# facebookresearch/FlowDec

Hardware: AMD Instinct MI355X
Metric: 48 kHz audio-seconds/sec (RTF) for FlowDec-75m @ 6 ODE steps (higher is better)
Workload: dtype bf16; 1 GPU; flowdec_75m enhance(): global batch=8 x 2 s clips @48 kHz (8 per GPU), 6-step euler (NFE 6), T_pad=256 frames, inputs resident in HBM, initial noise drawn inside the timed call, output waveforms all-gathered; global_batch=8, nfe=6, parallelism=batch-shard x1, hipgraph=True, conv_algo=auto

## Files before the change

flowdec_amd/csrc/conv_wino4.hip:

```cpp
#include <type_traits>

#include "conv_common.h"
#include "wino4_layout.h"

namespace {

using namespace fdconv;

typedef _Float16 f16;
typedef __attribute__((ext_vector_type(2))) _Float16 f16x2;
typedef __attribute__((ext_vector_type(8))) _Float16 f16x8;
typedef unsigned int u32x2 __attribute__((ext_vector_type(2)));
typedef float f32x2 __attribute__((ext_vector_type(2)));

constexpr int cmax(int a, int b) { return a > b ? a : b; }

using fdw4::NTH, fdw4::HH, fdw4::HW, fdw4::RROW, fdw4::RROW_BYTES, fdw4::RAW_PASSES, fdw4::RAW_BYTES, fdw4::NPIECE, fdw4::VXI;
constexpr int TH = 16, TW = 16, BN = 256;
static_assert(HH == TH + 2 && HW == TW + 2, "wino4_layout.h describes this tile");
constexpr int CK = 16;
constexpr int SLAB = BN * 32;
constexpr int RSLOT = 2048, NRING = 6;
static_assert(18 % NRING == 0, "the two-chunk loop body turns the ring a whole number of times");
constexpr int RING_BYTES = 8 * NRING * RSLOT;
constexpr int V_BYTES = 6 * VXI;
constexpr int V_OFF = RING_BYTES;
constexpr int AFF_OFF = V_OFF + 2 * V_BYTES;
constexpr int RAW_OFF = AFF_OFF + AFF_BYTES;
constexpr int MAIN_BYTES = RAW_OFF + RAW_BYTES;
constexpr int X_BYTES = 8 * 8192;
constexpr int S_PITCH = 128 * 4 + 16;
constexpr int S_BYTES = 128 * S_PITCH;
constexpr int SK_OFF = S_BYTES, SK_BYTES = 4 * NTH * 16;
constexpr int SCK = 2, SCD = 3;
constexpr int WS_BYTES = SCK * SLAB;
constexpr int XS_OFF = SCD * WS_BYTES, XS_BYTES = SCK * 8192;
constexpr int BIAS_OFF = 2 * S_BYTES;
static_assert(BIAS_OFF >= 2 * X_BYTES && BIAS_OFF >= SK_OFF + 2 * SK_BYTES && XS_OFF + SCD * XS_BYTES <= 160 * 1024, "epilogue LDS map");
constexpr int ISC_OFF = BIAS_OFF + 1024;
constexpr int STAT_OFF = ISC_OFF + 1024;
constexpr int LDS_BYTES = cmax(MAIN_BYTES, STAT_OFF + 16384);
static_assert(LDS_BYTES <= 160 * 1024 && NPIECE <= RAW_PASSES * NTH && AFF_BYTES <= 4 * 1024 && RAW_OFF % 128 == 0, "LDS layout");
constexpr int U_EXP = 9;
constexpr float RAW_MAX = 6000.f;

__device__ __forceinline__ unsigned pack_f16(float a, float b) {
  f16x2 r = {(f16)a, (f16)b};
  return __builtin_bit_cast(unsigned, r);
}
__device__ __forceinline__ f16x2 h2(unsigned u) { return __builtin_bit_cast(f16x2, u); }
__device__ __forceinline__ unsigned u2(f16x2 v) { return __builtin_bit_cast(unsigned, v); }

__device__ __forceinline__ void glds16s(const void* sbase, unsigned voff, unsigned lds_dst) {
  asm volatile("s_mov_b32 m0, %2\n\ts_nop 0\n\tglobal_load_lds_dwordx4 %0, %1" ::"v"(voff), "s"(sbase), "s"(lds_dst) : "memory");
}
__device__ __forceinline__ void glds16s_x2(const void* sbase, unsigned voff, unsigned lds_dst) {
  asm volatile("s_mov_b32 m0, %2\n\ts_nop 0\n\tglobal_load_lds_dwordx4 %0, %1\n\tglobal_load_lds_dwordx4 %0, %1 offset:1024" ::"v"(voff), "s"(sbase), "s"(lds_dst)
               : "memory");
}

template <bool ACT, bool SKIP, bool SC>
__global__ __launch_bounds__(NTH, 2) void conv_wino4_kernel(ConvArgs p) {
  static_assert(!(SKIP && SC), "residual input and folded shortcut exclude each other in this kernel");
  extern __shared__ __attribute__((aligned(16))) char smem[];
  FD_T2(const unsigned long long t2_entry = __builtin_amdgcn_s_memtime();)

  const int bid = blockIdx.x, nblk = gridDim.x;
  int lid;
  {
    const int xcd = bid & 7, qq = nblk >> 3, rr = nblk & 7;
    lid = (xcd < rr ? xcd * (qq + 1) : rr * (qq + 1) + (xcd - rr) * qq) + (bid >> 3);
  }
  if (p.reversed) lid = nblk - 1 - lid;
  int pt = lid;
  const int tw_i = pt % p.tiles_w; pt /= p.tiles_w;
  const int th_i = pt % p.tiles_h;
  const int b = pt / p.tiles_h;
  const int h0 = th_i * TH, w0 = tw_i * TW;
  const int H = p.H, W = p.W;

  const int t = threadIdx.x;
  const int lane = t & 63;
  const int wave = __builtin_amdgcn_readfirstlane(t >> 6);
  const int cq = wave & 3, xt = wave >> 2;

  auto opaque = [&](int v) { asm volatile("" : "+v"(v)); return v; };
  const size_t img_elems = (size_t)H * W;
  const int hb = h0 > 0 ? h0 - 1 : 0;
  const size_t band_pix = (size_t)b * img_elems + (size_t)hb * W;
  const bf16* const sb0 = reinterpret_cast<const bf16*>(p.seg[0].src) + band_pix * p.seg[0].C;
  const bool two3 = p.nseg > 1 && p.seg[1].taps == 9;
  const bf16* const sb1 = two3 ? reinterpret_cast<const bf16*>(p.seg[1].src) + band_pix * p.seg[1].C : sb0;
  const int sC0 = p.seg[0].C, sC1 = two3 ? p.seg[1].C : 0;
  const int nch0 = sC0 / CK, n3 = nch0 + sC1 / CK;
  int hpix[RAW_PASSES];
#pragma unroll
  for (int i = 0; i < RAW_PASSES; ++i) {
    const fdw4::Req rq = fdw4::raw_request(t + i * NTH);
    const int gh = h0 - 1 + rq.row, gw = w0 - 1 + rq.col;
    const bool ok = rq.col >= 0 && gh >= 0 && gh < H && gw >= 0 && gw < W;
    hpix[i] = ((ok ? (gh - hb) * W + gw : 0) << 2) | (ok ? rq.piece : t & 3);
  }
  int pA, vbits, pword;
  {
    const fdw4::Item it = fdw4::item(t);
    pA = fdw4::raw_addr(it.row, 6 * it.k, 0, it.word) | (fdw4::v_addr(it.row, fdw4::first_tile(it.k), it.word) << 16);
    const int gh = h0 - 1 + it.row;
    vbits = (it.k != 0 || w0 > 0 ? 1 : 0) | (gh >= 0 && gh < H ? 2 : 0) | (it.k != 2 || w0 + TW < W ? 4 : 0) | (it.active ? 8 : 0) |
            (it.active && it.k == 1 ? 16 : 0);
    pword = it.word;
  }
  const bf16* nbase = sb0;
  int nC2 = 0, ncb = 0;
  int cnext = 0;
  auto next_chunk = [&]() {
    if (cnext < n3) {
      const bool first = cnext < nch0;
      const int cch = first ? cnext : cnext - nch0;
      nbase = first ? sb0 : sb1;
      nC2 = (first ? sC0 : sC1) * 2;
      ncb = cch * CK * 2;
    }
    ++cnext;
  };
  const unsigned rawdst = (unsigned)(RAW_OFF + wave * 1024);
  auto load_halo = [&]() {
    const int on = cnext <= n3 ? 1 : 0;
#pragma unroll
    for (int i = 0; i < RAW_PASSES; ++i) {
      const int hp = opaque(hpix[i]);
      glds16s(nbase, (unsigned)(((hp >> 2) * nC2 + ncb + (hp & 3) * 16) * on), rawdst + i * 8192);
    }
  };
  int affa = AFF_OFF + pword * 16;
  auto load_affine = [&]() {
    if constexpr (ACT) {
      if (wave < AFF_BYTES / 1024) {
        const int o = opaque(t) * 16;
        glds16s(p.affine + (size_t)b * p.affC * 2, (unsigned)(o < n3 * CK * 8 ? o : 0), (unsigned)(AFF_OFF + wave * 1024));
      }
    }
  };

  auto produce = [&](const int e, const int vbuf, const int affo) {
    const int pa = opaque(pA), vbt = opaque(vbits);
    const char* const rp = smem + RAW_OFF + ((pa & 0xffff) ^ (e << 5));
    char* const vb = smem + V_OFF + vbuf * V_BYTES + (int)((unsigned)pa >> 16);
    unsigned w_[6];
#pragma unroll
    for (int j = 0; j < 6; ++j) w_[j] = *reinterpret_cast<const unsigned*>(rp + j * 64);
    f32x4 af = {0.f, 0.f, 0.f, 0.f};
    if constexpr (ACT) af = *reinterpret_cast<const f32x4*>(smem + opaque(affa) + affo);
    const unsigned mrow = (unsigned)((int)((unsigned)vbt << 30) >> 31);
    const unsigned m0 = mrow & (unsigned)((int)((unsigned)vbt << 31) >> 31), m5 = mrow & (unsigned)((int)((unsigned)vbt << 29) >> 31);
#pragma unroll
    for (int j = 0; j < 6; ++j) {
      const unsigned u = w_[j];
      const float x0 = __builtin_bit_cast(float, u << 16), x1 = __builtin_bit_cast(float, u & 0xffff0000u);
      unsigned r;
      if constexpr (ACT) {
        const f16x2 zc = {(f16)RAW_MAX, (f16)RAW_MAX};
        r = u2(__builtin_elementwise_min(h2(pack_f16(fd_silu(fmaf(x0, af[0], af[1])), fd_silu(fmaf(x1, af[2], af[3])))), zc));
      } else
        r = pack_f16(__builtin_amdgcn_fmed3f(x0, -RAW_MAX, RAW_MAX), __builtin_amdgcn_fmed3f(x1, -RAW_MAX, RAW_MAX));
      w_[j] = r & (j == 0 ? m0 : j == 5 ? m5 : mrow);
    }
    const unsigned l4 = (unsigned)__builtin_amdgcn_update_dpp(0, (int)w_[4], 0x111, 0xf, 0xf, true);
    const unsigned l5 = (unsigned)__builtin_amdgcn_update_dpp(0, (int)w_[5], 0x111, 0xf, 0xf, true);
    const unsigned r0 = (unsigned)__builtin_amdgcn_update_dpp(0, (int)w_[0], 0x101, 0xf, 0xf, true);
    const unsigned r1 = (unsigned)__builtin_amdgcn_update_dpp(0, (int)w_[1], 0x101, 0xf, 0xf, true);
    const bool mid = (vbt & 16) != 0;
    const f16x2 c4 = {(f16)4.f, (f16)4.f}, cm4 = {(f16)-4.f, (f16)-4.f}, cm5 = {(f16)-5.f, (f16)-5.f}, c2 = {(f16)2.f, (f16)2.f},
                cm2 = {(f16)-2.f, (f16)-2.f};
    auto transform = [&](char* const v, const unsigned d0, const unsigned d1, const unsigned d2, const unsigned d3, const unsigned d4, const unsigned d5) {
      const f16x2 z0 = h2(d0), z1 = h2(d1), z2 = h2(d2), z3 = h2(d3), z4 = h2(d4), z5 = h2(d5);
      const f16x2 t1 = __builtin_elementwise_fma(z2, cm4, z4);
      const f16x2 t2 = __builtin_elementwise_fma(z1, cm4, z3);
      const f16x2 t3 = z4 - z2, t4 = z3 - z1;
      *reinterpret_cast<unsigned*>(v + 0 * VXI) = u2(__builtin_elementwise_fma(z0, c4, __builtin_elementwise_fma(z2, cm5, z4)));
      *reinterpret_cast<unsigned*>(v + 1 * VXI) = u2(t1 + t2);
      *reinterpret_cast<unsigned*>(v + 2 * VXI) = u2(t1 - t2);
      *reinterpret_cast<unsigned*>(v + 4 * VXI) = u2(__builtin_elementwise_fma(t4, c2, t3));
      *reinterpret_cast<unsigned*>(v + 5 * VXI) = u2(__builtin_elementwise_fma(t4, cm2, t3));
      *reinterpret_cast<unsigned*>(v + 3 * VXI) = u2(__builtin_elementwise_fma(z1, c4, __builtin_elementwise_fma(z3, cm5, z5)));
    };
    if (vbt & 8)
      transform(vb, mid ? l4 : w_[0], mid ? l5 : w_[1], mid ? w_[0] : w_[2], mid ? w_[1] : w_[3], mid ? w_[2] : w_[4], mid ? w_[3] : w_[5]);
    if (mid) transform(vb + 32, w_[2], w_[3], w_[4], w_[5], r0, r1);
  };

  const char* wp = reinterpret_cast<const char*>(p.w) + (size_t)xt * 9 * SLAB + cq * 2048;
  asm volatile("" : "+s"(wp));
  const unsigned lane16 = (unsigned)(lane * 16);
  const unsigned wring = (unsigned)(wave * NRING * RSLOT);
  auto dma_step = [&](int f, int slot) {
    glds16s_x2(wp + (f / 9) * 18 * SLAB + (f % 9) * SLAB, lane16, wring + slot * RSLOT);
  };

  const int l31 = lane & 31, lh = lane >> 5;
  const int wa_lane = (int)wring + l31 * 32 + ((lh ^ ((l31 >> 3) & 1)) * 16);
  const int vb0 = V_OFF + xt * 3 * VXI  + l31 * 32 + ((lh ^ ((l31 >> 3) & 1)) * 16);
  const int vb1 = (vb0 ^ ((l31 & 4) << 2)) + 128;

  f32x16 acc[3][2][2];
#pragma unroll
  for (int x = 0; x < 3; ++x)
#pragma unroll
    for (int ct = 0; ct < 2; ++ct)
#pragma unroll
      for (int nt = 0; nt < 2; ++nt)
#pragma unroll
        for (int e = 0; e < 16; ++e) acc[x][ct][nt][e] = 0.f;

  auto lds_wait = [&]() { asm volatile("s_waitcnt lgkmcnt(0)" ::: "memory"); };
  auto barrier = [&]() {
    __builtin_amdgcn_s_barrier();
    asm volatile("" ::: "memory");
  };

  u32x4 qa[3], qb[3];
  auto mma = [&](int xl, int ct, int nt, const u32x4& a, const u32x4& bq) {
    acc[xl][ct][nt] = __builtin_amdgcn_mfma_f32_32x32x16_f16(__builtin_bit_cast(f16x8, a), __builtin_bit_cast(f16x8, bq), acc[xl][ct][nt], 0, 0, 0);
  };
  auto rd = [&](int off) { return *reinterpret_cast<const u32x4*>(smem + off); };
  auto a_off = [&](int k18, int ct) { return wa_lane + (k18 % NRING) * RSLOT + ct * 1024; };
  auto b_off = [&](int k18, int nt) {
    const int s = k18 % 9, half = (k18 / 9) & 1;
    const int dy = s % 3;
    return (dy == 0 ? vb0 : dy == 1 ? vb1 : (vb0 ^ 16) + 256) + half * V_BYTES + (s / 3) * VXI + nt * 1024;
  };

  next_chunk();
  load_halo();
  load_affine();
#pragma unroll
  for (int k = 0; k < NRING; ++k) dma_step(k, k);
  asm volatile("s_waitcnt vmcnt(0)" ::: "memory");
  barrier();
  produce(0, 0, 0);
  next_chunk();
  lds_wait();
  barrier();
  FD_T2(const unsigned long long t2_first = __builtin_amdgcn_s_memtime();)
  qa[0] = rd(a_off(0, 0)); qb[0] = rd(b_off(0, 0)); qb[1] = rd(b_off(0, 1)); qa[1] = rd(a_off(0, 1));

  constexpr int NW = 2 * (NRING - 2);
  for (int c = 0; c < n3; c += 2) {
    int xg = xt;
    asm volatile("" : "+s"(xg));
#pragma clang loop unroll(full)
    for (int k = 0; k < 18; ++k) {
      const int s = k % 9, half = k / 9;
      const int vn = half ^ 1;
      const int xl = s / 3;
      u32x4 &A0 = qa[(2 * k) % 3], &A1 = qa[(2 * k + 1) % 3], &A2 = qa[(2 * k + 2) % 3];
      u32x4 &B0 = qb[(2 * k) % 3], &B1 = qb[(2 * k + 1) % 3], &B2 = qb[(2 * k + 2) % 3];
      if (s >= 4 && s <= 7 && half == 0) asm volatile("s_waitcnt vmcnt(%0)" ::"n"(NW + RAW_PASSES) : "memory");
      else asm volatile("s_waitcnt vmcnt(%0)" ::"n"(NW) : "memory");
      if (s == 8 || (s == 3 && half == 0)) { lds_wait(); barrier(); }
      A2 = rd(a_off(k + 1, 0));
      B2 = rd(b_off(k + 1, 0));
      __builtin_amdgcn_sched_barrier(0);
      mma(xl, 0, 0, A0, B0);
      mma(xl, 0, 1, A0, B1);
      __builtin_amdgcn_sched_barrier(0);
      A0 = rd(a_off(k + 1, 1));
      mma(xl, 1, 0, A1, B0);
      __builtin_amdgcn_sched_barrier(0);
      B0 = rd(b_off(k + 1, 1));
      if (s == 3) { next_chunk(); if (half == 0) load_halo(); }
      dma_step(k + NRING, k % NRING);
      mma(xl, 1, 1, A1, B1);
      __builtin_amdgcn_sched_barrier(0);
      if (s == 0) { if (xg == 0) produce(half ^ 1, vn, 128 * (1 + half)); }
      if (s == 1) { if (xg == 1) produce(half ^ 1, vn, 128 * (1 + half)); }
      __builtin_amdgcn_sched_barrier(0);
    }
    wp += 36 * SLAB;
    asm volatile("" : "+s"(wp));
    affa += 2 * CK * 8;
  }
  asm volatile("s_waitcnt vmcnt(0)" ::: "memory");
  __syncthreads();
  FD_T2(const unsigned long long t2_loop = __builtin_amdgcn_s_memtime();)

  const size_t row0_pix = (size_t)b * img_elems + (size_t)h0 * W;
  bf16* const out = reinterpret_cast<bf16*>(p.out) + row0_pix * p.Cout;
  const bf16* const skip = SKIP ? reinterpret_cast<const bf16*>(p.skip) + row0_pix * p.Cout : nullptr;
  float* const biast = reinterpret_cast<float*>(smem + BIAS_OFF);
  float* const statt = reinterpret_cast<float*>(smem + STAT_OFF);
  float* const isct = reinterpret_cast<float*>(smem + ISC_OFF);
  auto load_bias_table = [&]() {
    if (t < BN) {
      biast[t] = p.bias ? p.bias[(size_t)(p.bias_rows > 1 ? b : 0) * p.Cout + t] * p.scale : 0.f;
      isct[t] = p.w_scale[t] * p.scale;
    }
  };
  if constexpr (!SC) load_bias_table();
  auto out_off = [&](int tt, int ct, int nt, int ps) {
    const int oct = tt & 15, pp = tt >> 4;
    const int rh = nt * 8 + (pp >> 2), gw = w0 + 4 * (pp & 3) + ps;
    return (rh * W + gw) * p.Cout + ct * 128 + oct * 8;
  };
  auto skip_dma = [&](int r) {
    if constexpr (SKIP) {
      const int tt = opaque(t);
#pragma unroll
      for (int ps = 0; ps < 4; ++ps)
        glds16s(skip, (unsigned)(out_off(tt, r >> 1, r & 1, ps) * 2), (unsigned)(SK_OFF + (r & 1) * SK_BYTES + ps * NTH * 16 + wave * 1024));
    }
  };
  skip_dma(0);
  skip_dma(1);
  FD_T2(
  unsigned long long t2_r[5] = {0, 0, 0, 0, 0};
  t2_r[0] = __builtin_amdgcn_s_memtime();
  )

  const float ka = xt ? 0.f : 1.f, ks = xt ? 4.f : 1.f, kb = xt ? 1.f : 0.f, kd = xt ? 8.f : 1.f, kq = xt ? 0.25f : 1.f;
  auto e1_round = [&](int rd_, int xoff) {
    const int ct = rd_ >> 1, nt = rd_ & 1;
    f32x16 &m0 = acc[0][ct][nt], &m1 = acc[1][ct][nt], &m2 = acc[2][ct][nt];
    const f32x2 kd2 = {kd, kd}, kq2 = {kq, kq}, ka2 = {ka, ka}, ks2 = {ks, ks}, kb2 = {kb, kb};
    char* const xmine = smem + xoff + wave * 8192 + lane * 16;
    const char* const xpeer = smem + xoff + (wave ^ 4) * 8192 + lane * 16;
#pragma unroll
    for (int g = 0; g < 4; ++g) {
      f32x2 snd[2];
#pragma unroll
      for (int h = 0; h < 2; ++h) {
        const int e = 4 * g + 2 * h;
        const f32x2 a1 = {m1[e], m1[e + 1]}, a2 = {m2[e], m2[e + 1]};
        const f32x2 s_ = a1 + a2, d_ = (a1 - a2) * kd2;
        m2[e] = s_[0]; m2[e + 1] = s_[1];
        m1[e] = d_[0]; m1[e + 1] = d_[1];
        snd[h] = d_ * kq2;
      }
      *reinterpret_cast<f32x4*>(xmine + g * 1024) = f32x4{m2[4 * g], m2[4 * g + 1], m2[4 * g + 2], m2[4 * g + 3]};
      *reinterpret_cast<f32x4*>(xmine + 4096 + g * 1024) = f32x4{snd[0][0], snd[0][1], snd[1][0], snd[1][1]};
    }
    lds_wait();
    barrier();
#pragma unroll
    for (int g = 0; g < 4; ++g) {
      const f32x4 r0 = *reinterpret_cast<const f32x4*>(xpeer + g * 1024), r1 = *reinterpret_cast<const f32x4*>(xpeer + 4096 + g * 1024);
#pragma unroll
      for (int h = 0; h < 2; ++h) {
        const int e = 4 * g + 2 * h;
        const f32x2 mm = {m0[e], m0[e + 1]}, ss = {m2[e], m2[e + 1]}, dd = {m1[e], m1[e + 1]};
        const f32x2 q0 = {r0[2 * h], r0[2 * h + 1]}, q1 = {r1[2 * h], r1[2 * h + 1]};
        const f32x2 ya = __builtin_elementwise_fma(ka2, mm, __builtin_elementwise_fma(ks2, ss, q0));
        const f32x2 yb = __builtin_elementwise_fma(kb2, mm, dd + q1);
        m0[e] = ya[0]; m0[e + 1] = ya[1];
        m1[e] = yb[0]; m1[e + 1] = yb[1];
      }
    }
  };
  float ssum[8], ssq[8];
  auto e3_round = [&](int rd_, int soff) {
    const int ct = rd_ >> 1, nt = rd_ & 1;
    f32x16 &m0 = acc[0][ct][nt], &m1 = acc[1][ct][nt];
    char* const sbuf = smem + soff;
    if (nt == 0) {
#pragma unroll
      for (int j = 0; j < 8; ++j) ssum[j] = ssq[j] = 0.f;
    }
    {
      char* const sbase = sbuf + ((2 * xt) * 32 + l31) * S_PITCH + (cq * 32 + 4 * lh) * 4;
#pragma unroll
      for (int g = 0; g < 4; ++g) {
        *reinterpret_cast<f32x4*>(sbase + g * 32) = f32x4{m0[4 * g], m0[4 * g + 1], m0[4 * g + 2], m0[4 * g + 3]};
        *reinterpret_cast<f32x4*>(sbase + 32 * S_PITCH + g * 32) = f32x4{m1[4 * g], m1[4 * g + 1], m1[4 * g + 2], m1[4 * g + 3]};
      }
    }
    lds_wait();
    barrier();
    __builtin_amdgcn_sched_barrier(0);
    if constexpr (SKIP) {
      if (rd_ == 0 || rd_ == 3) asm volatile("s_waitcnt vmcnt(4)" ::: "memory");
      else asm volatile("s_waitcnt vmcnt(8)" ::: "memory");
    }
    {
      const int tt = opaque(t);
      const int oct = tt & 15, pp = tt >> 4;
      const f32x4 bA = *reinterpret_cast<const f32x4*>(biast + ct * 128 + oct * 8), bB = *reinterpret_cast<const f32x4*>(biast + ct * 128 + oct * 8 + 4);
      const float bv[8] = {bA[0], bA[1], bA[2], bA[3], bB[0], bB[1], bB[2], bB[3]};
      const f32x4 iA = *reinterpret_cast<const f32x4*>(isct + ct * 128 + oct * 8), iB = *reinterpret_cast<const f32x4*>(isct + ct * 128 + oct * 8 + 4);
      const float iv[8] = {iA[0], iA[1], iA[2], iA[3], iB[0], iB[1], iB[2], iB[3]};
#pragma unroll
      for (int bt = 0; bt < 2; ++bt) {
        u32x4 packed[2];
        int ooff[2];
#pragma unroll
        for (int q = 0; q < 2; ++q) {
          const int ps = 2 * bt + q;
          ooff[q] = out_off(tt, ct, nt, ps);
          const float* sp = reinterpret_cast<const float*>(sbuf + (pp + ps * 32) * S_PITCH) + oct * 8;
          const f32x4 v0 = *reinterpret_cast<const f32x4*>(sp), v1 = *reinterpret_cast<const f32x4*>(sp + 4);
          float v[8] = {v0[0], v0[1], v0[2], v0[3], v1[0], v1[1], v1[2], v1[3]};
          if constexpr (SKIP) {
            const u32x4 skr = *reinterpret_cast<const u32x4*>(smem + SK_OFF + (rd_ & 1) * SK_BYTES + (ps * NTH + tt) * 16);
            const bf16x8 sk = __builtin_bit_cast(bf16x8, skr);
#pragma unroll
            for (int k = 0; k < 4; ++k) {
              const f32x2 s2_ = {(float)sk[2 * k], (float)sk[2 * k + 1]}, sc2 = {p.scale, p.scale}, b2 = {bv[2 * k], bv[2 * k + 1]};
              const f32x2 i2 = {iv[2 * k], iv[2 * k + 1]}, x_ = {v[2 * k], v[2 * k + 1]};
              const f32x2 r_ = __builtin_elementwise_fma(x_, i2, __builtin_elementwise_fma(s2_, sc2, b2));
              v[2 * k] = r_[0]; v[2 * k + 1] = r_[1];
            }
          }
#pragma unroll
          for (int k = 0; k < 4; ++k) {
#pragma clang fp contract(off)
            f32x2 x = {v[2 * k], v[2 * k + 1]};
            f32x2 s1 = {ssum[2 * k], ssum[2 * k + 1]}, s2 = {ssq[2 * k], ssq[2 * k + 1]};
            if constexpr (!SKIP) {
              const f32x2 b2 = {bv[2 * k], bv[2 * k + 1]}, i2 = {iv[2 * k], iv[2 * k + 1]};
              x = __builtin_elementwise_fma(x, i2, b2);
            }
            s1 += x;
            s2 = __builtin_elementwise_fma(x, x, s2);
            v[2 * k] = x[0]; v[2 * k + 1] = x[1];
            ssum[2 * k] = s1[0]; ssum[2 * k + 1] = s1[1];
            ssq[2 * k] = s2[0]; ssq[2 * k + 1] = s2[1];
          }
          bf16x8 tv;
#pragma unroll
          for (int j = 0; j < 8; ++j) tv[j] = (bf16)v[j];
          packed[q] = __builtin_bit_cast(u32x4, tv);
        }
#pragma unroll
        for (int q = 0; q < 2; ++q) *reinterpret_cast<u32x4*>(out + ooff[q]) = packed[q];
      }
    }
    if (nt == 1 && p.stats) {
#pragma unroll
      for (int j = 0; j < 8; ++j) {
        ssum[j] += __shfl_xor(ssum[j], 16, 64); ssq[j] += __shfl_xor(ssq[j], 16, 64);
        ssum[j] += __shfl_xor(ssum[j], 32, 64); ssq[j] += __shfl_xor(ssq[j], 32, 64);
      }
      if (lane < 16) {
        float* rec = statt + ((ct * 8 + wave) * 16 + lane) * 16;
#pragma unroll
        for (int j = 0; j < 4; ++j) *reinterpret_cast<f32x4*>(rec + 4 * j) = f32x4{ssum[2 * j], ssq[2 * j], ssum[2 * j + 1], ssq[2 * j + 1]};
      }
    }
  };

  if constexpr (SC) {
#pragma unroll
    for (int rd_ = 0; rd_ < 4; ++rd_) {
      e1_round(rd_, (rd_ & 1) * X_BYTES);
      __builtin_amdgcn_sched_barrier(0);
    }
    lds_wait();
    barrier();
    FD_T2(t2_r[1] = __builtin_amdgcn_s_memtime();)
    {
      const int nsc = p.nseg - (sC1 ? 2 : 1);
      const Seg q0 = p.seg[p.nseg - nsc], q1 = p.seg[p.nseg - 1];
      const int S0 = q0.C, Stot = S0 + (nsc > 1 ? q1.C : 0);
      const int nstage = Stot / (16 * SCK);
      const bf16* const xb0 = reinterpret_cast<const bf16*>(q0.src) + row0_pix * q0.C;
      const bf16* const xb1 = reinterpret_cast<const bf16*>(q1.src) + row0_pix * q1.C;
      const char* const wsc = reinterpret_cast<const char*>(p.w) + (size_t)(n3 + 1) * 18 * SLAB + cq * 2048;
      static_assert(SCK == 2, "a stage row = 2 K steps x 2 halves x 16 B; K step kk of the weights is loaded by wave group xt = kk");
      int xsrc[2];
#pragma unroll
      for (int i = 0; i < 2; ++i) {
        const int r = ((i * 8 + wave) * 64 + lane) >> 2;
        const int xtile = r & 63, xj = r >> 6;
        const int piece = (lane & 3) ^ ((r >> 2) & 3);
        xsrc[i] = (((xtile >> 2) * W + w0 + 4 * (xtile & 3) + xj) << 8) | (piece * 16);
      }
      const unsigned lane16e = (unsigned)(lane * 16);
      auto stage_dma = [&](int st, int slot) {
        const int ste = st < nstage ? st : 0;
        const int c0 = ste * 16 * SCK;
        const bool first = c0 < S0;
        const bf16* const xb = first ? xb0 : xb1;
        const int Cs = first ? S0 : Stot - S0, cc = first ? c0 : c0 - S0;
#pragma unroll
        for (int i = 0; i < 2; ++i)
          glds16s(xb, (unsigned)(((xsrc[i] >> 8) * Cs + cc) * 2 + (xsrc[i] & 255)), (unsigned)(XS_OFF + slot * XS_BYTES + i * 8192 + wave * 1024));
        glds16s_x2(wsc + (size_t)(ste * SCK + xt) * SLAB, lane16e, (unsigned)(slot * WS_BYTES + xt * SLAB + cq * 2048));
      };
      const int wa_sc = cq * 2048 + l31 * 32 + ((lh ^ ((l31 >> 3) & 1)) * 16);
      const int xb_row = XS_OFF + ((2 * xt) * 64 + l31) * 64;
      const int xb_sw = (l31 >> 2) & 3;
#pragma unroll
      for (int d = 0; d < SCD - 1; ++d) stage_dma(d, d);
      int slot = 0;
      for (int st = 0; st < nstage; ++st) {
        asm volatile("s_waitcnt vmcnt(%0)" ::"n"(4 * (SCD - 2)) : "memory");
        lds_wait();
        barrier();
        const int nslot = slot == 0 ? SCD - 1 : slot - 1;
        stage_dma(st + SCD - 1, nslot);
        const int wo = slot * WS_BYTES, xo = slot * XS_BYTES;
        u32x4 af[SCK][2], bq[SCK][2][2];
#pragma unroll
        for (int kk = 0; kk < SCK; ++kk) {
          af[kk][0] = rd(wa_sc + wo + kk * SLAB);
          af[kk][1] = rd(wa_sc + wo + kk * SLAB + 1024);
#pragma unroll
          for (int pl = 0; pl < 2; ++pl)
#pragma unroll
            for (int nt = 0; nt < 2; ++nt) bq[kk][pl][nt] = rd(xb_row + xo + (pl * 64 + nt * 32) * 64 + (((kk * 2 + lh) ^ xb_sw) * 16));
        }
        __builtin_amdgcn_sched_barrier(0);
#pragma unroll
        for (int kk = 0; kk < SCK; ++kk)
#pragma unroll
          for (int pl = 0; pl < 2; ++pl)
#pragma unroll
            for (int nt = 0; nt < 2; ++nt) {
              acc[pl][0][nt] = __builtin_amdgcn_mfma_f32_32x32x16_bf16(__builtin_bit_cast(bf16x8, af[kk][0]), __builtin_bit_cast(bf16x8, bq[kk][pl][nt]), acc[pl][0][nt], 0, 0, 0);
              acc[pl][1][nt] = __builtin_amdgcn_mfma_f32_32x32x16_bf16(__builtin_bit_cast(bf16x8, af[kk][1]), __builtin_bit_cast(bf16x8, bq[kk][pl][nt]), acc[pl][1][nt], 0, 0, 0);
            }
        __builtin_amdgcn_sched_barrier(0);
        slot = slot + 1 == SCD ? 0 : slot + 1;
      }
      asm volatile("s_waitcnt vmcnt(0)" ::: "memory");
      lds_wait();
      barrier();
      load_bias_table();
    }
    FD_T2(t2_r[2] = __builtin_amdgcn_s_memtime();)
#pragma unroll
    for (int rd_ = 0; rd_ < 4; ++rd_) {
      e3_round(rd_, (rd_ & 1) * S_BYTES);
      __builtin_amdgcn_sched_barrier(0);
    }
  } else {
#pragma unroll
    for (int rd_ = 0; rd_ < 4; ++rd_) {
      e1_round(rd_, 0);
      if constexpr (SKIP) { lds_wait(); barrier(); }
      e3_round(rd_, SKIP ? 0 : X_BYTES);
      if constexpr (SKIP) {
        lds_wait();
        barrier();
        if (rd_ < 2) skip_dma(rd_ + 2);
      }
      __builtin_amdgcn_sched_barrier(0);
    }
  }
  FD_T2(t2_r[3] = __builtin_amdgcn_s_memtime();)
  if (p.stats) {
    lds_wait();
    barrier();
    const int ch = t >> 1, which = t & 1;
    const int ct = ch >> 7, oc = (ch >> 3) & 15, j = ch & 7;
    const float* src = statt + (ct * 8 * 16 + oc) * 16 + 2 * j + which;
    float a = 0.f;
#pragma unroll
    for (int w_ = 0; w_ < 8; ++w_) a += src[w_ * 256];
    const int tile = th_i * p.tiles_w + tw_i;
    p.stats[((size_t)b * p.tiles_h * p.tiles_w + tile) * p.CoutPad * 2 + t] = a;
  }
  FD_T2(
  if (p.dbg && t == 0 && bid < 8192) {
    const unsigned long long t2_end = __builtin_amdgcn_s_memtime();
    unsigned long long* d = p.dbg + (size_t)bid * 8;
    d[0] = t2_first - t2_entry; d[1] = t2_loop - t2_first; d[2] = t2_end - t2_loop;
    d[3] = t2_r[1] - t2_r[0]; d[4] = t2_r[2] - t2_r[1]; d[5] = t2_r[3] - t2_r[2]; d[6] = t2_end - t2_r[3]; d[7] = t2_r[0] - t2_loop;
  }
  )
}

__device__ __forceinline__ float wino4_u(const float* g, int xi) {
  const float g0 = g[0], g1 = g[1], g2 = g[2];
  switch (xi) {
    case 0: return 0.25f * g0;
    case 1: return -(g0 + g1 + g2) / 6.f;
    case 2: return (-g0 + g1 - g2) / 6.f;
    case 3: return g0 / 24.f + g1 / 12.f + g2 / 6.f;
    case 4: return g0 / 24.f - g1 / 12.f + g2 / 6.f;
    default: return g2;
  }
}

constexpr int SC_EXP_MAX = 60;
__global__ void wino4_scale_kernel(const float* __restrict__ w, const float* __restrict__ w_sc, float* __restrict__ tab, int Cout, int Cin, int S) {
  __shared__ float red[256], red_sc[256];
  const int co = blockIdx.x, t = threadIdx.x;
  float m = 0.f, msc = 0.f;
  if (co < Cout) {
    for (int i = t; i < Cin * 3; i += 256) {
      const float* g = w + ((size_t)co * Cin * 3 + i) * 3;
#pragma unroll
      for (int xi = 0; xi < 6; ++xi) m = fmaxf(m, fabsf(wino4_u(g, xi)));
    }
    if (w_sc)
      for (int i = t; i < S; i += 256) msc = fmaxf(msc, fabsf(w_sc[(size_t)co * S + i]));
  }
  red[t] = m;
  red_sc[t] = msc;
  __syncthreads();
  for (int o = 128; o > 0; o >>= 1) {
    if (t < o) { red[t] = fmaxf(red[t], red[t + o]); red_sc[t] = fmaxf(red_sc[t], red_sc[t + o]); }
    __syncthreads();
  }
  if (t == 0) {
    int k = 0;
    m = red[0];
    msc = red_sc[0];
    if (m > 0.f && m < 3.0e38f) {
      int e;
      frexpf(m, &e);
      k = U_EXP - e;
      k = k < -100 ? -100 : (k > 100 ? 100 : k);
      if (msc > 0.f && msc < 3.0e38f) {
        int es;
        frexpf(msc, &es);
        if (k > SC_EXP_MAX - es) k = SC_EXP_MAX - es;
      }
    }
    tab[co] = ldexpf(1.f, -k);
    tab[BN + co] = ldexpf(1.f, k);
  }
}

__global__ void wino4_pack_kernel(const float* __restrict__ w, f16* __restrict__ dst, const float* __restrict__ tab, int Cout, int C0, int C1) {
  const int Cin = C0 + C1, nchunks = Cin / CK;
  const long long total = (long long)nchunks * 18 * BN * CK;
  for (long long i = blockIdx.x * (long long)blockDim.x + threadIdx.x; i < total; i += (long long)gridDim.x * blockDim.x) {
    const int k = (int)(i % CK);
    long long r = i / CK;
    const int n = (int)(r % BN); r /= BN;
    const int dy = (int)(r % 3); r /= 3;
    const int slot = (int)(r % 6);
    const int xi = slot < 3 ? slot : (slot == 3 ? 5 : slot - 1);
    const int chunk = (int)(r / 6);
    const int c = chunk * CK + k;
    const int co = ((n >> 5) & 1) * 128 + (n >> 6) * 32 + (n & 31);
    float v = 0.f;
    if (co < Cout) v = wino4_u(w + (((size_t)co * Cin + c) * 3 + dy) * 3, xi) * tab[BN + co];
    const int half = (k >> 3) ^ ((n >> 3) & 1);
    dst[(i - k) + half * 8 + (k & 7)] = (f16)v;
  }
}

__global__ void wino4_pack_sc_kernel(const float* __restrict__ w, bf16* __restrict__ dst, const float* __restrict__ tab, int Cout, int S) {
  const long long total = (long long)(S / CK) * BN * CK;
  for (long long i = blockIdx.x * (long long)blockDim.x + threadIdx.x; i < total; i += (long long)gridDim.x * blockDim.x) {
    const int k = (int)(i % CK);
    long long r = i / CK;
    const int n = (int)(r % BN);
    const int ks = (int)(r / BN);
    const int co = ((n >> 5) & 1) * 128 + (n >> 6) * 32 + (n & 31);
    const float v = co < Cout ? w[(size_t)co * S + ks * CK + k] * tab[BN + co] : 0.f;
    const int half = (k >> 3) ^ ((n >> 3) & 1);
    dst[(i - k) + half * 8 + (k & 7)] = (bf16)v;
  }
}

}

bool fd_wino4_supported(int Cout, int C0, int C1, int S0, int S1, int ksize) {
  return ksize == 3 && Cout == BN && C0 > 0 && C0 % 32 == 0 && C1 % 32 == 0 && S0 % 32 == 0 && S1 % 32 == 0 && (S1 == 0 || S0 > 0) &&
         (C0 + C1) * 8 <= AFF_BYTES;
}
bool fd_wino4_shape_ok(int H, int W) { return H % TH == 0 && W % TW == 0; }

namespace {
constexpr long long W4_HDR = 4096;
}

long long fd_wino4_packed_bytes(int Cout, int C0, int C1, int S0, int S1) {
  (void)Cout;
  return W4_HDR + (long long)((C0 + C1) / CK + 1) * 18 * SLAB + (long long)((S0 + S1) / CK) * SLAB + 16 * 1024;
}

int fd_wino4_pack_weights(const float* w, const float* w_sc, void* packed, int Cout, int C0, int C1, int S0, int S1, hipStream_t st) {
  const long long total = (long long)((C0 + C1) / CK) * 18 * BN * CK;
  const int blocks = (int)((total + 255) / 256 > 4096 ? 4096 : (total + 255) / 256);
  float* const tab = reinterpret_cast<float*>(packed);
  char* const steps = reinterpret_cast<char*>(packed) + W4_HDR;
  hipLaunchKernelGGL(wino4_scale_kernel, dim3(BN), dim3(256), 0, st, w, w_sc, tab, Cout, C0 + C1, w_sc ? S0 + S1 : 0);
  hipLaunchKernelGGL(wino4_pack_kernel, dim3(blocks), dim3(256), 0, st, w, (f16*)steps, tab, Cout, C0, C1);
  if (w_sc) {
    const long long tsc = (long long)((S0 + S1) / CK) * BN * CK;
    const int bsc = (int)((tsc + 255) / 256 > 4096 ? 4096 : (tsc + 255) / 256);
    hipLaunchKernelGGL(wino4_pack_sc_kernel, dim3(bsc), dim3(256), 0, st, w_sc,
                       reinterpret_cast<bf16*>(steps + (size_t)((C0 + C1) / CK + 1) * 18 * SLAB), tab, Cout, S0 + S1);
  }
  FD_LAUNCH_CHECK();
  return FD_OK;
}

namespace {
template <bool ACT>
int set_attr4() {
  FD_HIP(hipFuncSetAttribute(reinterpret_cast<const void*>(conv_wino4_kernel<ACT, false, false>), hipFuncAttributeMaxDynamicSharedMemorySize, LDS_BYTES));
  FD_HIP(hipFuncSetAttribute(reinterpret_cast<const void*>(conv_wino4_kernel<ACT, true, false>), hipFuncAttributeMaxDynamicSharedMemorySize, LDS_BYTES));
  FD_HIP(hipFuncSetAttribute(reinterpret_cast<const void*>(conv_wino4_kernel<ACT, false, true>), hipFuncAttributeMaxDynamicSharedMemorySize, LDS_BYTES));
  return FD_OK;
}
template <bool ACT>
void launch4(const ConvArgs& a, bool sc, dim3 grid, dim3 block, hipStream_t st) {
  if (sc) hipLaunchKernelGGL((conv_wino4_kernel<ACT, false, true>), grid, block, LDS_BYTES, st, a);
  else if (a.skip) hipLaunchKernelGGL((conv_wino4_kernel<ACT, true, false>), grid, block, LDS_BYTES, st, a);
  else hipLaunchKernelGGL((conv_wino4_kernel<ACT, false, false>), grid, block, LDS_BYTES, st, a);
}
}

int fd_wino4_init_attributes() {
  FD_TRY(set_attr4<false>());
  FD_TRY(set_attr4<true>());
  return FD_OK;
}

int fd_wino4_launch(ConvArgs a, hipStream_t st) {
  FD_REQUIRE(fd_wino4_shape_ok(a.H, a.W), "fd_conv2d: FD_WINOGRAD4 needs H %% 16 == 0 and W %% 16 == 0 (got %d x %d)", a.H, a.W);
  bool sc = false;
  for (int s = 0; s < a.nseg; ++s) sc = sc || a.seg[s].taps == 1;
  a.w_scale = reinterpret_cast<const float*>(a.w);
  a.w = reinterpret_cast<const char*>(a.w) + W4_HDR;
  FD_REQUIRE(!(sc && a.skip), "fd_conv2d: FD_WINOGRAD4 takes a folded shortcut or a residual input, not both");
  a.tiles_h = a.H / TH;
  a.tiles_w = a.W / TW;
  a.tiles_n = 1;
  a.CoutPad = BN;
  const long long nblk = (long long)a.B * a.tiles_h * a.tiles_w;
  FD_REQUIRE(nblk > 0 && nblk < (1ll << 31), "conv grid out of range");
  const dim3 grid((unsigned)nblk), block(NTH);
  if (a.affine) launch4<true>(a, sc, grid, block, st);
  else launch4<false>(a, sc, grid, block, st);
  FD_LAUNCH_CHECK();
  return FD_OK;
}
```

Before: 132.9 audio-seconds/second.

## Halve Winograd output-transform LDS exchange by refactoring butterfly across wave pairs

Rewrites the cross-wave stage of the Winograd output transform. Each wave now keeps one butterfly combination in registers and sends only the other to its peer wave, so the LDS exchange buffer per wave is halved and one f32x4 store and load per group is dropped. The coefficients are refactored into sign and scale constants, and the output-row mapping (xt*32 vs 2*xt*32, and the 64-row offset in the stats staging and the shortcut B-fragment reads) is changed to match the new ownership of rows. The risk is numerical or row-mapping mismatch if the new coefficients or layout are not exactly equivalent to the old ones.

```diff
diff --git a/flowdec_amd/csrc/conv_wino4.hip b/flowdec_amd/csrc/conv_wino4.hip
--- a/flowdec_amd/csrc/conv_wino4.hip
+++ b/flowdec_amd/csrc/conv_wino4.hip
@@ -28,7 +28,8 @@
 constexpr int AFF_OFF = V_OFF + 2 * V_BYTES;
 constexpr int RAW_OFF = AFF_OFF + AFF_BYTES;
 constexpr int MAIN_BYTES = RAW_OFF + RAW_BYTES;
-constexpr int X_BYTES = 8 * 8192;
+constexpr int X_WAVE = 4 * 64 * 16;
+constexpr int X_BYTES = 8 * X_WAVE;
 constexpr int S_PITCH = 128 * 4 + 16;
 constexpr int S_BYTES = 128 * S_PITCH;
 constexpr int SK_OFF = S_BYTES, SK_BYTES = 4 * NTH * 16;
@@ -36,7 +37,8 @@
 constexpr int WS_BYTES = SCK * SLAB;
 constexpr int XS_OFF = SCD * WS_BYTES, XS_BYTES = SCK * 8192;
 constexpr int BIAS_OFF = 2 * S_BYTES;
-static_assert(BIAS_OFF >= 2 * X_BYTES && BIAS_OFF >= SK_OFF + 2 * SK_BYTES && XS_OFF + SCD * XS_BYTES <= 160 * 1024, "epilogue LDS map");
+static_assert(BIAS_OFF >= 2 * X_BYTES && BIAS_OFF >= X_BYTES + S_BYTES && BIAS_OFF >= SK_OFF + 2 * SK_BYTES && XS_OFF + SCD * XS_BYTES <= 160 * 1024,
+              "epilogue LDS map");
 constexpr int ISC_OFF = BIAS_OFF + 1024;
 constexpr int STAT_OFF = ISC_OFF + 1024;
 constexpr int LDS_BYTES = cmax(MAIN_BYTES, STAT_OFF + 16384);
@@ -317,13 +319,13 @@
   t2_r[0] = __builtin_amdgcn_s_memtime();
   )
 
-  const float ka = xt ? 0.f : 1.f, ks = xt ? 4.f : 1.f, kb = xt ? 1.f : 0.f, kd = xt ? 8.f : 1.f, kq = xt ? 0.25f : 1.f;
+  const float sg = xt ? -1.f : 1.f, ka = xt ? 0.f : 1.f, kb = xt ? 1.f : 0.f, cka = xt ? 2.f : 1.f, ckb = xt ? 8.f : 1.f, cr = xt ? 1.f : 4.f;
   auto e1_round = [&](int rd_, int xoff) {
     const int ct = rd_ >> 1, nt = rd_ & 1;
     f32x16 &m0 = acc[0][ct][nt], &m1 = acc[1][ct][nt], &m2 = acc[2][ct][nt];
-    const f32x2 kd2 = {kd, kd}, kq2 = {kq, kq}, ka2 = {ka, ka}, ks2 = {ks, ks}, kb2 = {kb, kb};
-    char* const xmine = smem + xoff + wave * 8192 + lane * 16;
-    const char* const xpeer = smem + xoff + (wave ^ 4) * 8192 + lane * 16;
+    const f32x2 sg2 = {sg, sg}, ka2 = {ka, ka}, kb2 = {kb, kb}, cka2 = {cka, cka}, ckb2 = {ckb, ckb}, cr2 = {cr, cr};
+    char* const xmine = smem + xoff + wave * X_WAVE + lane * 16;
+    const char* const xpeer = smem + xoff + (wave ^ 4) * X_WAVE + lane * 16;
 #pragma unroll
     for (int g = 0; g < 4; ++g) {
       f32x2 snd[2];
@@ -331,26 +333,24 @@
       for (int h = 0; h < 2; ++h) {
         const int e = 4 * g + 2 * h;
         const f32x2 a1 = {m1[e], m1[e + 1]}, a2 = {m2[e], m2[e + 1]};
-        const f32x2 s_ = a1 + a2, d_ = (a1 - a2) * kd2;
-        m2[e] = s_[0]; m2[e + 1] = s_[1];
-        m1[e] = d_[0]; m1[e + 1] = d_[1];
-        snd[h] = d_ * kq2;
-      }
-      *reinterpret_cast<f32x4*>(xmine + g * 1024) = f32x4{m2[4 * g], m2[4 * g + 1], m2[4 * g + 2], m2[4 * g + 3]};
-      *reinterpret_cast<f32x4*>(xmine + 4096 + g * 1024) = f32x4{snd[0][0], snd[0][1], snd[1][0], snd[1][1]};
+        const f32x2 keep = __builtin_elementwise_fma(sg2, a2, a1);
+        snd[h] = __builtin_elementwise_fma(-sg2, a2, a1);
+        m2[e] = keep[0]; m2[e + 1] = keep[1];
+      }
+      *reinterpret_cast<f32x4*>(xmine + g * 1024) = f32x4{snd[0][0], snd[0][1], snd[1][0], snd[1][1]};
     }
     lds_wait();
     barrier();
 #pragma unroll
     for (int g = 0; g < 4; ++g) {
-      const f32x4 r0 = *reinterpret_cast<const f32x4*>(xpeer + g * 1024), r1 = *reinterpret_cast<const f32x4*>(xpeer + 4096 + g * 1024);
+      const f32x4 r0 = *reinterpret_cast<const f32x4*>(xpeer + g * 1024);
 #pragma unroll
       for (int h = 0; h < 2; ++h) {
         const int e = 4 * g + 2 * h;
-        const f32x2 mm = {m0[e], m0[e + 1]}, ss = {m2[e], m2[e + 1]}, dd = {m1[e], m1[e + 1]};
-        const f32x2 q0 = {r0[2 * h], r0[2 * h + 1]}, q1 = {r1[2 * h], r1[2 * h + 1]};
-        const f32x2 ya = __builtin_elementwise_fma(ka2, mm, __builtin_elementwise_fma(ks2, ss, q0));
-        const f32x2 yb = __builtin_elementwise_fma(kb2, mm, dd + q1);
+        const f32x2 mm = {m0[e], m0[e + 1]}, kp = {m2[e], m2[e + 1]};
+        const f32x2 r = {r0[2 * h], r0[2 * h + 1]}, rr = cr2 * r;
+        const f32x2 ya = __builtin_elementwise_fma(ka2, mm, __builtin_elementwise_fma(cka2, kp, r));
+        const f32x2 yb = __builtin_elementwise_fma(kb2, mm, __builtin_elementwise_fma(ckb2, kp, rr));
         m0[e] = ya[0]; m0[e + 1] = ya[1];
         m1[e] = yb[0]; m1[e + 1] = yb[1];
       }
@@ -366,11 +366,11 @@
       for (int j = 0; j < 8; ++j) ssum[j] = ssq[j] = 0.f;
     }
     {
-      char* const sbase = sbuf + ((2 * xt) * 32 + l31) * S_PITCH + (cq * 32 + 4 * lh) * 4;
+      char* const sbase = sbuf + (xt * 32 + l31) * S_PITCH + (cq * 32 + 4 * lh) * 4;
 #pragma unroll
       for (int g = 0; g < 4; ++g) {
         *reinterpret_cast<f32x4*>(sbase + g * 32) = f32x4{m0[4 * g], m0[4 * g + 1], m0[4 * g + 2], m0[4 * g + 3]};
-        *reinterpret_cast<f32x4*>(sbase + 32 * S_PITCH + g * 32) = f32x4{m1[4 * g], m1[4 * g + 1], m1[4 * g + 2], m1[4 * g + 3]};
+        *reinterpret_cast<f32x4*>(sbase + 64 * S_PITCH + g * 32) = f32x4{m1[4 * g], m1[4 * g + 1], m1[4 * g + 2], m1[4 * g + 3]};
       }
     }
     lds_wait();
@@ -486,7 +486,7 @@
         glds16s_x2(wsc + (size_t)(ste * SCK + xt) * SLAB, lane16e, (unsigned)(slot * WS_BYTES + xt * SLAB + cq * 2048));
       };
       const int wa_sc = cq * 2048 + l31 * 32 + ((lh ^ ((l31 >> 3) & 1)) * 16);
-      const int xb_row = XS_OFF + ((2 * xt) * 64 + l31) * 64;
+      const int xb_row = XS_OFF + (xt * 64 + l31) * 64;
       const int xb_sw = (l31 >> 2) & 3;
 #pragma unroll
       for (int d = 0; d < SCD - 1; ++d) stage_dma(d, d);
@@ -506,7 +506,7 @@
 #pragma unroll
           for (int pl = 0; pl < 2; ++pl)
 #pragma unroll
-            for (int nt = 0; nt < 2; ++nt) bq[kk][pl][nt] = rd(xb_row + xo + (pl * 64 + nt * 32) * 64 + (((kk * 2 + lh) ^ xb_sw) * 16));
+            for (int nt = 0; nt < 2; ++nt) bq[kk][pl][nt] = rd(xb_row + xo + (pl * 128 + nt * 32) * 64 + (((kk * 2 + lh) ^ xb_sw) * 16));
         }
         __builtin_amdgcn_sched_barrier(0);
 #pragma unroll
```

After: 133.8 audio-seconds/second, median of 6. No clear change (+0.7%).
